# shenwei356/LexicMap

Measured on NVIDIA B200. Metric: aligned query bp/s, higher is better.
Workload: dtype int64

## Files before the change

lexicmap_b200/csrc/engine.cu:

```cuda
#include "image.cuh"
#include "../../include/lexicmap_gpu.h"
#include <cub/cub.cuh>
#include <cmath>
#include <cfloat>
#include <algorithm>
#include <numeric>
#include <chrono>
#include <mutex>
#include <atomic>
#include <thread>
#include <condition_variable>
#include <functional>
#include <exception>
#include <set>
#include <array>
#include <memory>
#include <sched.h>

#define FULLMASK 0xffffffffu
static std::atomic<unsigned long long> g_launches{0};
#undef KERNEL_CHECK
#define KERNEL_CHECK() do { g_launches++; CUDA_CHECK(cudaGetLastError()); } while (0)
#define CUB_CHECK() CUDA_CHECK(cudaGetLastError())
static inline int cdiv(i64 a, i64 b) { return (int)((a + b - 1) / b); }
// ... 838 lines not shown
    if (lane == 0) {
      R.wscore = s; i32 k = kend, off = tlen, sc = s; int mat = 0; i32 vv = off - k, h = off; u64* ops = (u64*)(slab + ((used + 1) & ~1ull)); u64 ops_room = (slab_words - ((used + 1) & ~1ull)) / 2; u32 nops = 0; bool ops_over = false;
      int cur = 0; u32 curn = 0; i32 p_alen = 0, p_gaps = 0, p_bs = 0; int prev = 0;
      auto flush = [&]() { if (want_ops && curn) { if (nops < ops_room) ops[nops++] = ((u64)cur << 32) | curn; else ops_over = true; } curn = 0; };
      auto put = [&](int op, i32 cntp, i32 vend, i32 hend) {
        if (cntp <= 0) return; if (op != cur) { flush(); cur = op; } curn += (u32)cntp;
        if (op == 'M') { if (R.has_m) { R.alen += p_alen; R.gaps += p_gaps; R.bscore += p_bs; } else { R.has_m = 1; R.qend = vend; R.tend = hend; } p_alen = p_gaps = p_bs = 0; R.alen += cntp; R.matches += cntp; R.bscore += 2 * cntp; R.qbegin = vend - cntp + 1; R.tbegin = hend - cntp + 1; }
        else if (op == 'X') { p_alen += cntp; p_bs -= 3 * cntp; } else { p_alen += cntp; p_gaps += cntp; p_bs -= 2 * cntp; if (prev != op) p_bs -= 5; }
        prev = op; };
      while (vv > 0 && h > 0 && sc > 0) {
        i32 s_mis = sc - X, s_open = sc - OE, s_ext = sc - E; i64 c_mis = INT64_MIN, c_io = INT64_MIN, c_ie = INT64_MIN, c_do = INT64_MIN, c_de = INT64_MIN;
        auto pig = [](i32 o, int type) -> i64 { return o <= WF_NULL ? INT64_MIN : (((i64)o << 4) | type); };
        if (mat == 0) { i32 o = (s_mis >= 0) ? getw(s_mis / STEP, 0, k) : WF_NULL; c_mis = pig(o <= WF_NULL ? WF_NULL : o + 1, 9); }
        if (mat == 0 || mat == 1) { i32 o = (s_open >= 0) ? getw(s_open / STEP, 0, k - 1) : WF_NULL; c_io = pig(o <= WF_NULL ? WF_NULL : o + 1, 1); o = (s_ext >= 0) ? getw(s_ext / STEP, 1, k - 1) : WF_NULL; c_ie = pig(o <= WF_NULL ? WF_NULL : o + 1, 2); }
        if (mat == 0 || mat == 2) { c_do = pig((s_open >= 0) ? getw(s_open / STEP, 0, k + 1) : WF_NULL, 5); c_de = pig((s_ext >= 0) ? getw(s_ext / STEP, 2, k + 1) : WF_NULL, 6); }
        i64 best = max(c_mis, max(max(c_io, c_ie), max(c_do, c_de))); if (best == INT64_MIN) { R.status = 2; break; }
        if (mat == 0) { i32 mo = (i32)(best >> 4); i32 nm = off - mo; put('M', nm, off - k, off); off = mo; vv = off - k; h = off; if (vv <= 0 || h <= 0) continue; }
        int type = (int)(best & 15);
        switch (type) { case 9: sc = s_mis; mat = 0; put('X', 1, off - k, off); off--; break;
          case 1: sc = s_open; mat = 0; put('I', 1, off - k, off); k--; off--; break; case 2: sc = s_ext; mat = 1; put('I', 1, off - k, off); k--; off--; break;
          case 5: sc = s_open; mat = 0; put('D', 1, off - k, off); k++; break; case 6: sc = s_ext; mat = 2; put('D', 1, off - k, off); k++; break; }
        vv = off - k; h = off;
      }
      if (R.status == 0) { if (sc == 0) put('M', off, off - k, off); else { if (vv > 0) put('D', vv, vv, h); if (h > 0) put('I', h, 0, h); } }
      flush();
      if (want_ops && R.status == 0) { if (ops_over) R.status = 1; else { u64 o = atomicAdd((unsigned long long*)ops_cursor, (unsigned long long)nops); if (o + nops <= ops_cap) { for (u32 i = 0; i < nops; i++) ops_pool[o + i] = ops[i]; R.ops_off = o; R.ops_n = nops; } else R.status = 3; } }
      outs[jb] = R;
    }
    __syncwarp();
  }
}

#define WF_WMAX 256
#define WF_PAD 8
#define WFS (WF_WMAX + 2 * WF_PAD)
#define WFK0 (WF_WMAX / 2 + WF_PAD)
#define WF_LMAX 2048
#define WF_OPSMAX 4096
#define WF_WARPS 8
#define WF_SEQW 144
#define X2_LV 2
#define OE2_LV 4
#define E2_LV 1
#define WF_SMEM_BYTES ((size_t)WF_WARPS * (WF_SEQW * 8 + 9 * WFS * 2 + WFS * 2))
struct WfaSeg { u64 qw, tw; };

__global__ void k_wfa_prep(const HspJob* __restrict__ jobs, const ExtOut* __restrict__ ext, u32 njobs, const u64* __restrict__ woff , const u8* __restrict__ qpacked, const u8* __restrict__ qamask, const u64* __restrict__ qboff,
                           const u8* __restrict__ g2bit, const u64* __restrict__ g_off, u64* __restrict__ words, u32* __restrict__ has_amb) {
  u32 jb = blockIdx.x; if (jb >= njobs) return; if (threadIdx.x == 0) has_amb[jb] = 0; __syncthreads(); HspJob J = jobs[jb]; ExtOut e = ext[jb]; const u8* q2 = qpacked + qboff[J.q]; const u8* qm = qamask + qboff[J.q]; const u8* g2 = g2bit + g_off[J.g];
  i32 plen = e.qe - e.qs, tlen = e.te - e.ts; u32 nq = (u32)((plen + 31) / 32 + 2), nt = (u32)((tlen + 31) / 32 + 2); u64* Q = words + woff[2 * jb]; u64* A = Q + nq; u64* T = words + woff[2 * jb + 1];
  for (u32 w = threadIdx.x; w < nq; w += blockDim.x) { u64 b = 0, a = 0; for (int j = 0; j < 32; j++) { i32 i = (i32)w * 32 + j; u64 c = 0, am = 0; if (i < plen) { i32 p = e.qs + i; c = get_base(q2, (u64)p); am = ((qm[p >> 3] >> (p & 7)) & 1) ? 3 : 0; } b = (b << 2) | c; a = (a << 2) | am; } Q[w] = b; A[w] = a; if (a) has_amb[jb] = 1; }
  for (u32 w = threadIdx.x; w < nt; w += blockDim.x) { u64 b = 0; for (int j = 0; j < 32; j++) { i32 i = (i32)w * 32 + j; u64 c = (i < tlen) ? win_base(g2, J.tBegin, J.tEnd, J.rc, e.ts + i) : 0; b = (b << 2) | c; } T[w] = b; }
}
__device__ __forceinline__ u64 fetch64(const u64* __restrict__ W, i32 pos) { u32 i = (u32)pos >> 5, sh = ((u32)pos & 31) * 2; u64 a = W[i]; if (sh == 0) return a; return (a << sh) | (W[i + 1] >> (64 - sh)); }

__global__ void __launch_bounds__(WF_WARPS * 32) k_wfa_fast(const ExtOut* __restrict__ ext, const u64* __restrict__ woff, const u64* __restrict__ words, const u32* __restrict__ has_amb, const u32* __restrict__ job_ids, u32 job0, u32 njobs, u32* __restrict__ next_job,
                                                          u16* __restrict__ slabs, WfaOut* __restrict__ outs, int adaptive, int lmax) {
  extern __shared__ __align__(16) u8 wf_smem[];
  const int X2 = 2, OE2 = 4, E2 = 1;
  int lane = threadIdx.x & 31, wib = threadIdx.x >> 5; u64* seqb = (u64*)wf_smem + (size_t)wib * WF_SEQW; u16 (*R)[WFS] = (u16 (*)[WFS])(wf_smem + (size_t)WF_WARPS * WF_SEQW * 8) + (size_t)wib * 9;
  u16* Dst = (u16*)(wf_smem + (size_t)WF_WARPS * WF_SEQW * 8 + (size_t)WF_WARPS * 9 * WFS * 2) + (size_t)wib * WFS;
  for (;;) {
    u32 jr = 0; if (lane == 0) jr = atomicAdd(next_job, 1u); jr = __shfl_sync(FULLMASK, jr, 0); if (jr >= njobs) return; const u32 jb = job_ids ? job_ids[job0 + jr] : job0 + jr; u16* slab = slabs + (u64)jr * lmax * 3 * WFS;
    ExtOut ex = ext[jb]; const i32 plen = ex.qe - ex.qs, tlen = ex.te - ex.ts, kend = tlen - plen; const u32 nqw = (u32)((plen + 31) / 32 + 2);
    const u64* Q = words + woff[2 * jb]; const u64* A = Q + nqw; const u64* T = words + woff[2 * jb + 1]; const bool amb = has_amb[jb] != 0;
    {
      const u32 ntw = (u32)((tlen + 31) / 32 + 2), nA = amb ? nqw : 0; __syncwarp();
      if (nqw + nA + ntw <= WF_SEQW) { u64* sq = seqb; for (u32 i = lane; i < nqw + nA; i += 32) sq[i] = Q[i]; for (u32 i = lane; i < ntw; i += 32) sq[nqw + nA + i] = T[i]; __syncwarp(); Q = sq; A = sq + nqw; T = sq + nqw + nA; } }
    WfaOut Rz; Rz.qbegin = Rz.qend = Rz.tbegin = Rz.tend = Rz.alen = Rz.matches = Rz.gaps = Rz.bscore = Rz.has_m = 0; Rz.wscore = 0; Rz.status = 0; Rz.ops_n = 0; Rz.ops_off = 0;
    if (plen >= 32000 || tlen >= 32000 || kend <= -(WF_WMAX / 2) + 2 || kend >= WF_WMAX / 2 - 2 || plen <= 0 || tlen <= 0) { if (lane == 0) { Rz.status = 1; outs[jb] = Rz; } __syncwarp(); continue; }
    auto extend = [&](i32 k, i32 h) { i32 v = h - k; for (;;) { i32 rem = min(plen - v, tlen - h); if (rem <= 0) break; u64 x = fetch64(Q, v) ^ fetch64(T, h); if (amb) x |= fetch64(A, v); i32 n = x ? (__clzll(x) >> 1) : 32; n = min(n, rem); v += n; h += n; if (n < 32) break; } return h; };
    i32 hlo[4], hhi[4]; u32 hnull[4]; for (int i = 0; i < 4; i++) { hlo[i] = 0; hhi[i] = -1; hnull[i] = 7; }
    for (int t = lane; t < 9 * WFS / 2; t += 32) ((u32*)&R[0][0])[t] = 0xFFFFFFFFu; __syncwarp();
    { i32 h0 = 0; if (lane == 0) h0 = extend(0, 0); h0 = __shfl_sync(FULLMASK, h0, 0);
      for (i32 k = -WF_PAD + lane; k <= WF_PAD; k += 32) { u16 mv = (k == 0) ? (u16)h0 : (u16)0xFFFF; R[0][k + WFK0] = mv; slab[k + WFK0] = mv; slab[WFS + k + WFK0] = 0xFFFF; slab[2 * WFS + k + WFK0] = 0xFFFF; R[5][k + WFK0] = 0xFFFF; R[7][k + WFK0] = 0xFFFF; }
      hlo[0] = 0; hhi[0] = 0; hnull[0] = 6; __syncwarp(); }
    i32 L = 0; bool done = (kend == 0 && R[0][WFK0] != 0xFFFF && (i32)R[0][WFK0] >= tlen), overflow = false;
    while (!done) {
      L++; if (L >= lmax) { overflow = true; break; }
      bool nx = (L - X2 < 0) || (hnull[X2 - 1] & 1), no = (L - OE2 < 0) || (hnull[OE2 - 1] & 1), ni = (hnull[E2 - 1] >> 1) & 1, nd = (hnull[E2 - 1] >> 2) & 1;
      i32 lo = INT32_MAX, hi = INT32_MIN; bool allnull = nx && no && ni && nd;
      if (!allnull) { if (!nx) { lo = min(lo, hlo[X2 - 1]); hi = max(hi, hhi[X2 - 1]); } if (!no) { lo = min(lo, hlo[OE2 - 1] - 1); hi = max(hi, hhi[OE2 - 1] + 1); } if (!ni || !nd) { lo = min(lo, hlo[E2 - 1] - 1); hi = max(hi, hhi[E2 - 1] + 1); } }
      i32 rlo = INT32_MAX, rhi = INT32_MIN; for (int i = 0; i < 4; i++) if (hnull[i] != 7) { rlo = min(rlo, hlo[i]); rhi = max(rhi, hhi[i]); }
      i32 wl = min(allnull ? INT32_MAX : lo, rlo), wh = max(allnull ? INT32_MIN : hi, rhi); if (wl > wh) { wl = 0; wh = 0; }
      if (wl <= -(WF_WMAX / 2) || wh >= WF_WMAX / 2) { overflow = true; break; }
      const u16* M2 = R[(L + 5 - X2) % 5]; const u16* M4 = R[(L + 5 - OE2) % 5]; const u16* I1 = R[5 + ((L + 1) & 1)]; const u16* D1 = R[7 + ((L + 1) & 1)];
      u16* Mo = R[L % 5]; u16* Io = R[5 + (L & 1)]; u16* Do = R[7 + (L & 1)]; u16* G = slab + (u64)L * 3 * WFS; bool anyM = false, anyI = false, anyD = false;
      u32 bitM = 0, bitI = 0, bitD = 0, itb = 1; i32 mind = INT32_MAX; const i32 k0 = wl - WF_PAD + lane;
      for (i32 k = k0; k <= wh + WF_PAD; k += 32, itb <<= 1) {
        u16 om = 0xFFFF, oi = 0xFFFF, od = 0xFFFF, dd = 0xFFFF; int x = k + WFK0;
        if (!allnull && k >= lo && k <= hi) {
          i32 ins = max((i32)(i16)M4[x - 1], (i32)(i16)I1[x - 1]); ins = (ins < 0) ? -1 : ins + 1;
          i32 del = max((i32)(i16)M4[x + 1], (i32)(i16)D1[x + 1]);
          i32 mis = (i32)(i16)M2[x]; mis = (mis < 0) ? -1 : mis + 1;
          const i32 hmax = min(tlen, plen + k);
          if (ins > hmax) ins = -1; if (del > hmax || del - k < 0) del = -1; if (mis > hmax) mis = -1;
          i32 mm = max(mis, max(ins, del)); if (mm >= 0) { mm = extend(k, mm); bitM |= itb; om = (u16)mm; i32 dv = max(plen - (mm - k), tlen - mm); dd = (u16)dv; mind = min(mind, dv); } if (ins >= 0) { bitI |= itb; oi = (u16)ins; } if (del >= 0) { bitD |= itb; od = (u16)del; }
        }
        Mo[x] = om; Io[x] = oi; Do[x] = od; Dst[x] = dd; G[x] = om; G[WFS + x] = oi; G[2 * WFS + x] = od;
      }
      anyM = __any_sync(FULLMASK, bitM != 0); anyI = __any_sync(FULLMASK, bitI != 0); anyD = __any_sync(FULLMASK, bitD != 0); __syncwarp();
      if (adaptive && !allnull && anyM && hi - lo + 1 >= 10) {
        for (int o = 16; o; o >>= 1) mind = min(mind, __shfl_xor_sync(FULLMASK, mind, o));
        const i32 thr = mind + 50; i32 top_limit = min(kend, hi); i32 nlo = lo; bool found = false;
        for (i32 b0 = lo; b0 < top_limit && !found; b0 += 32) { i32 k = b0 + lane; bool okk = (k < top_limit) && ((i32)Dst[k + WFK0] <= thr); u32 bal = __ballot_sync(FULLMASK, okk); if (bal) { nlo = b0 + __ffs(bal) - 1; found = true; } }
        if (!found && top_limit > lo) nlo = top_limit;
        i32 bottom_limit = max(kend, nlo); i32 nhi = hi; found = false;
        for (i32 b0 = hi; b0 > bottom_limit && !found; b0 -= 32) { i32 k = b0 - lane; bool okk = (k > bottom_limit) && ((i32)Dst[k + WFK0] <= thr); u32 bal = __ballot_sync(FULLMASK, okk); if (bal) { nhi = b0 - (__ffs(bal) - 1); found = true; } }
        if (!found && hi > bottom_limit) nhi = bottom_limit;
        if (nlo != lo || nhi != hi) { for (i32 k = lo + lane; k <= hi; k += 32) if (k < nlo || k > nhi) { int x = k + WFK0; Mo[x] = 0xFFFF; Io[x] = 0xFFFF; Do[x] = 0xFFFF; G[x] = 0xFFFF; G[WFS + x] = 0xFFFF; G[2 * WFS + x] = 0xFFFF; }
          i32 a0 = nlo - k0, a1 = nhi - k0; i32 itlo = a0 <= 0 ? 0 : (a0 + 31) >> 5, ithi = a1 < 0 ? -1 : (a1 >> 5); u32 keep = (ithi < itlo) ? 0u : ((ithi >= 31 ? 0xFFFFFFFFu : ((2u << ithi) - 1)) & ~((1u << itlo) - 1));
          anyM = __any_sync(FULLMASK, (bitM & keep) != 0); anyI = __any_sync(FULLMASK, (bitI & keep) != 0); anyD = __any_sync(FULLMASK, (bitD & keep) != 0); lo = nlo; hi = nhi; __syncwarp(); }
      }
      for (int i = 3; i > 0; i--) { hlo[i] = hlo[i - 1]; hhi[i] = hhi[i - 1]; hnull[i] = hnull[i - 1]; }
      hlo[0] = allnull ? 0 : lo; hhi[0] = allnull ? -1 : hi; hnull[0] = allnull ? 7u : ((anyM ? 0u : 1u) | (anyI ? 0u : 2u) | (anyD ? 0u : 4u));
      __syncwarp();
      if (!allnull && kend >= lo && kend <= hi) { u16 v = Mo[kend + WFK0]; done = (v != 0xFFFF && (i32)v >= tlen); }
    }
    if (lane == 0) { Rz.status = overflow ? 1 : 0; Rz.wscore = 2 * L; outs[jb] = Rz; }
    __syncwarp();
  }
}
__global__ void __launch_bounds__(128) k_wfa_bt(const ExtOut* __restrict__ ext, const u32* __restrict__ job_ids, u32 job0, u32 njobs, const u16* __restrict__ slabs, u64* __restrict__ ops_scratch, WfaOut* __restrict__ outs, u64* __restrict__ ops_pool, u64* __restrict__ ops_cursor, u64 ops_cap, int want_ops, int lmax) {
  const int X2 = 2, OE2 = 4, E2 = 1; u32 t = blockIdx.x * blockDim.x + threadIdx.x; if (t >= njobs) return; u32 jb = job_ids ? job_ids[job0 + t] : job0 + t; WfaOut Rr = outs[jb]; if (Rr.status != 0) return;
  ExtOut ex = ext[jb]; const i32 plen = ex.qe - ex.qs, tlen = ex.te - ex.ts, kend = tlen - plen; const u16* slab = slabs + (u64)t * lmax * 3 * WFS; u64* ops = ops_scratch + (u64)t * WF_OPSMAX;
  i32 L = Rr.wscore / 2; i32 k = kend, off = tlen, lv = L; int mat = 0; i32 vv = off - k, h = off; u32 nops = 0; bool ops_over = false; int cur = 0; u32 curn = 0; i32 p_alen = 0, p_gaps = 0, p_bs = 0; int prev = 0; (void)plen;
  auto flush = [&]() { if (want_ops && curn) { if (nops < WF_OPSMAX) ops[nops++] = ((u64)cur << 32) | curn; else ops_over = true; } curn = 0; };
  auto put = [&](int op, i32 cntp, i32 vend, i32 hend) { if (cntp <= 0) return; if (op != cur) { flush(); cur = op; } curn += (u32)cntp;
    if (op == 'M') { if (Rr.has_m) { Rr.alen += p_alen; Rr.gaps += p_gaps; Rr.bscore += p_bs; } else { Rr.has_m = 1; Rr.qend = vend; Rr.tend = hend; } p_alen = p_gaps = p_bs = 0; Rr.alen += cntp; Rr.matches += cntp; Rr.bscore += 2 * cntp; Rr.qbegin = vend - cntp + 1; Rr.tbegin = hend - cntp + 1; }
    else if (op == 'X') { p_alen += cntp; p_bs -= 3 * cntp; } else { p_alen += cntp; p_gaps += cntp; p_bs -= 2 * cntp; if (prev != op) p_bs -= 5; } prev = op; };
  auto ld = [&](i32 lvl, int comp, i32 kk) -> i32 { if (lvl < 0) return -1; u16 v = slab[(u64)lvl * 3 * WFS + comp * WFS + kk + WFK0]; return v == 0xFFFF ? -1 : (i32)v; };
  auto pig = [](i32 o, int type) -> i64 { return o < 0 ? INT64_MIN : (((i64)o << 4) | type); };
  while (vv > 0 && h > 0 && lv > 0) {
    i32 l_mis = lv - X2, l_open = lv - OE2, l_ext = lv - E2; i64 c_mis = INT64_MIN, c_io = INT64_MIN, c_ie = INT64_MIN, c_do = INT64_MIN, c_de = INT64_MIN;
    i32 v_mis = -1, v_io = -1, v_ie = -1, v_do = -1, v_de = -1;
    if (mat == 0) v_mis = ld(l_mis, 0, k); if (mat == 0 || mat == 1) { v_io = ld(l_open, 0, k - 1); v_ie = ld(l_ext, 1, k - 1); } if (mat == 0 || mat == 2) { v_do = ld(l_open, 0, k + 1); v_de = ld(l_ext, 2, k + 1); }
    if (mat == 0) c_mis = pig(v_mis < 0 ? -1 : v_mis + 1, 9); if (mat == 0 || mat == 1) { c_io = pig(v_io < 0 ? -1 : v_io + 1, 1); c_ie = pig(v_ie < 0 ? -1 : v_ie + 1, 2); } if (mat == 0 || mat == 2) { c_do = pig(v_do, 5); c_de = pig(v_de, 6); }
    i64 best = max(c_mis, max(max(c_io, c_ie), max(c_do, c_de))); if (best == INT64_MIN) { Rr.status = 2; break; }
    if (mat == 0) { i32 mo = (i32)(best >> 4); i32 nm = off - mo; put('M', nm, off - k, off); off = mo; vv = off - k; h = off; if (vv <= 0 || h <= 0) continue; }
    int type = (int)(best & 15);
    switch (type) { case 9: lv = l_mis; mat = 0; put('X', 1, off - k, off); off--; break;
      case 1: lv = l_open; mat = 0; put('I', 1, off - k, off); k--; off--; break; case 2: lv = l_ext; mat = 1; put('I', 1, off - k, off); k--; off--; break;
      case 5: lv = l_open; mat = 0; put('D', 1, off - k, off); k++; break; case 6: lv = l_ext; mat = 2; put('D', 1, off - k, off); k++; break; }
    vv = off - k; h = off;
  }
  if (Rr.status == 0) { if (lv == 0) put('M', off, off - k, off); else { if (vv > 0) put('D', vv, vv, h); if (h > 0) put('I', h, 0, h); } }
  flush();
  if (want_ops && Rr.status == 0) { if (ops_over) Rr.status = 1; else { u64 o = atomicAdd((unsigned long long*)ops_cursor, (unsigned long long)nops); if (o + nops <= ops_cap) { for (u32 i = 0; i < nops; i++) ops_pool[o + i] = ops[i]; Rr.ops_off = o; Rr.ops_n = nops; } else Rr.status = 3; } }
  outs[jb] = Rr;
}

#define WR_WARPS 8
#define WR_SEQW 144
#define WR_SMEM_BYTES ((size_t)WR_WARPS * WR_SEQW * 8)
#define WR_MAXLEN (1 << 20)
#define WR_NS 4
#define WR_W (32 * WR_NS)
struct WrCell { i32 om, oi, od, dv; u32 word; };
template <int NS>
__global__ void __launch_bounds__(WR_WARPS * 32) k_wfa_reg(const ExtOut* __restrict__ ext, const u64* __restrict__ woff, const u64* __restrict__ words, const u32* __restrict__ has_amb, const u32* __restrict__ job_ids, u32 job0, u32 njobs, u32* __restrict__ next_job,
                                                         u32* __restrict__ slabs, const u64* __restrict__ slab_off, WfaOut* __restrict__ outs, int adaptive) {
  extern __shared__ __align__(16) u8 wr_smem[];
  constexpr int W = 32 * NS;
  const int X2 = 2, OE2 = 4, E2 = 1; const int lane = threadIdx.x & 31, wib = threadIdx.x >> 5; u64* seqb = (u64*)wr_smem + (size_t)wib * WR_SEQW; const int lm1 = (lane + 31) & 31, lp1 = (lane + 1) & 31;
  for (;;) {
    u32 jr = 0; if (lane == 0) jr = atomicAdd(next_job, 1u); jr = __shfl_sync(FULLMASK, jr, 0); if (jr >= njobs) return; const u32 jb = job_ids ? job_ids[job0 + jr] : job0 + jr;
    u32* slab = slabs + slab_off[jr] * W; const i32 lmax = (i32)(slab_off[jr + 1] - slab_off[jr]);
    ExtOut ex = ext[jb]; const i32 plen = ex.qe - ex.qs, tlen = ex.te - ex.ts, kend = tlen - plen; const u32 nqw = (u32)((plen + 31) / 32 + 2);
    const u64* Q = words + woff[2 * jb]; const u64* A = Q + nqw; const u64* T = words + woff[2 * jb + 1]; const bool amb = has_amb[jb] != 0;
    { const u32 ntw = (u32)((tlen + 31) / 32 + 2), nA = amb ? nqw : 0; __syncwarp();
      if (nqw + nA + ntw <= WR_SEQW) { u64* sq = seqb; for (u32 i = lane; i < nqw + nA; i += 32) sq[i] = Q[i]; for (u32 i = lane; i < ntw; i += 32) sq[nqw + nA + i] = T[i]; __syncwarp(); Q = sq; A = sq + nqw; T = sq + nqw + nA; } }
    WfaOut Rz; Rz.qbegin = Rz.qend = Rz.tbegin = Rz.tend = Rz.alen = Rz.matches = Rz.gaps = Rz.bscore = Rz.has_m = 0; Rz.wscore = 0; Rz.status = 0; Rz.ops_n = 0; Rz.ops_off = 0;
    if (plen >= WR_MAXLEN || tlen >= WR_MAXLEN || plen <= 0 || tlen <= 0 || lmax < 2) { if (lane == 0) { Rz.status = 1; Rz.wscore = -3; outs[jb] = Rz; } __syncwarp(); continue; }
    auto extend = [&](i32 kk, i32 h) { i32 v = h - kk; for (;;) { i32 rem = min(plen - v, tlen - h); if (rem <= 0) break; u64 x = fetch64(Q, v) ^ fetch64(T, h); if (amb) x |= fetch64(A, v); i32 n = x ? (__clzll(x) >> 1) : 32; n = min(n, rem); v += n; h += n; if (n < 32) break; } return h; };
    auto cell = [&](i32 k, bool live, i32 c_m2, i32 m4l, i32 i1l, i32 m4r, i32 d1r) { WrCell c; c.om = -1; c.oi = -1; c.od = -1; c.dv = INT32_MAX; c.word = 0;
      if (live) { i32 ins = max(m4l, i1l); ins = (ins < 0) ? -1 : ins + 1; i32 del = max(m4r, d1r); i32 mis = (c_m2 < 0) ? -1 : c_m2 + 1;
        const i32 hmax = min(tlen, plen + k); if (ins > hmax) ins = -1; if (del > hmax || del - k < 0) del = -1; if (mis > hmax) mis = -1;
        i32 mm = max(mis, max(ins, del)); if (mm >= 0) { c.om = extend(k, mm); c.dv = max(plen - (c.om - k), tlen - c.om); } c.oi = ins; c.od = del;
        i32 best = -1; if (c_m2 >= 0) best = ((c_m2 + 1) << 4) | 9; if (m4l >= 0) best = max(best, ((m4l + 1) << 4) | 1); if (i1l >= 0) best = max(best, ((i1l + 1) << 4) | 2); if (m4r >= 0) best = max(best, (m4r << 4) | 5); if (d1r >= 0) best = max(best, (d1r << 4) | 6);
        if (best >= 0) c.word = (u32)(best >> 4) | ((u32)(best & 15) << 20);
        if (i1l >= 0 && i1l >= m4l) c.word |= 1u << 24; if (d1r >= 0 && d1r >= m4r) c.word |= 1u << 25; if (m4l < 0 && i1l < 0) c.word |= 1u << 26; if (m4r < 0 && d1r < 0) c.word |= 1u << 27; }
      return c; };
    i32 hlo[4], hhi[4]; u32 hnull[4]; for (int i = 0; i < 4; i++) { hlo[i] = 0; hhi[i] = -1; hnull[i] = 7; }
    i32 kb = -16;
    i32 m1[NS], m2[NS], m3[NS], m4[NS], i1[NS], d1[NS];
#pragma unroll
    for (int s_ = 0; s_ < NS; s_++) { m1[s_] = m2[s_] = m3[s_] = m4[s_] = i1[s_] = d1[s_] = -1; }
    if (kb + lane == 0) m1[0] = extend(0, 0); hlo[0] = 0; hhi[0] = 0; hnull[0] = 6; slab[lane] = lane == 0 ? (u32)kb : 0u;
    auto at = [&](const i32 (&v)[NS], i32 j) { i32 r = -1;
#pragma unroll
      for (int t = 0; t < NS; t++) { const i32 x = __shfl_sync(FULLMASK, v[t], j & 31); if ((j >> 5) == t) r = x; } return r; };
    i32 L = 0, why = 0; bool done = false, overflow = false; { const i32 v0 = at(m1, 0 - kb); done = (kend == 0 && v0 >= tlen); }
    while (!done) {
      L++; if (L >= lmax) { overflow = true; why = -1; break; }
      const bool nx = (L - X2 < 0) || (hnull[X2 - 1] & 1), no = (L - OE2 < 0) || (hnull[OE2 - 1] & 1), ni = (hnull[E2 - 1] >> 1) & 1, nd = (hnull[E2 - 1] >> 2) & 1;
      i32 lo = INT32_MAX, hi = INT32_MIN; const bool allnull = nx && no && ni && nd;
      if (!allnull) { if (!nx) { lo = min(lo, hlo[X2 - 1]); hi = max(hi, hhi[X2 - 1]); } if (!no) { lo = min(lo, hlo[OE2 - 1] - 1); hi = max(hi, hhi[OE2 - 1] + 1); } if (!ni || !nd) { lo = min(lo, hlo[E2 - 1] - 1); hi = max(hi, hhi[E2 - 1] + 1); } }
      i32 slo = allnull ? INT32_MAX : lo, shi = allnull ? INT32_MIN : hi; for (int i = 0; i < 4; i++) if (hnull[i] != 7) { slo = min(slo, hlo[i]); shi = max(shi, hhi[i]); }
      if (slo <= shi) { const i32 span = shi - slo + 1;
        if (slo < kb + 1 || shi > kb + W - 2 || (span <= 30 && shi > kb + 30)) { if (span > W - 2) { overflow = true; why = -2; break; }
          const i32 room = min(W - 2, ((span + 33) >> 5) * 32 - 2); const i32 nkb = slo - 1 - (room - span) / 2, dlt = nkb - kb;
          const int sl = (lane + (dlt & 31)) & 31, carry = (lane + (dlt & 31)) >> 5, q = dlt >> 5;
          auto shift = [&](i32 (&v)[NS]) { i32 x[NS];
#pragma unroll
            for (int t = 0; t < NS; t++) x[t] = __shfl_sync(FULLMASK, v[t], sl);
#pragma unroll
            for (int s_ = 0; s_ < NS; s_++) { const int src = s_ + q + carry; i32 r = -1;
#pragma unroll
              for (int t = 0; t < NS; t++) if (src == t) r = x[t]; v[s_] = r; } };
          shift(m1); shift(m2); shift(m3); shift(m4); shift(i1); shift(d1); kb = nkb; } }
      const int sa = (slo <= shi) ? max(0, (slo - kb) >> 5) : 0, sb = (slo <= shi) ? min(NS - 1, (shi - kb) >> 5) : -1;
      WrCell c[NS];
#pragma unroll
      for (int s_ = 0; s_ < NS; s_++) { c[s_].om = c[s_].oi = c[s_].od = -1; c[s_].dv = INT32_MAX; c[s_].word = 0; }
      if (!allnull) {
        i32 r4[NS], ri[NS], t4[NS], td[NS];
#pragma unroll
        for (int t = 0; t < NS; t++) { r4[t] = ri[t] = t4[t] = td[t] = -1; if (t >= sa && t <= sb) { r4[t] = __shfl_sync(FULLMASK, m4[t], lm1); ri[t] = __shfl_sync(FULLMASK, i1[t], lm1); t4[t] = __shfl_sync(FULLMASK, m4[t], lp1); td[t] = __shfl_sync(FULLMASK, d1[t], lp1); } }
#pragma unroll
        for (int s_ = 0; s_ < NS; s_++) if (s_ >= sa && s_ <= sb && lo <= kb + 32 * s_ + 31 && hi >= kb + 32 * s_) { const i32 k = kb + 32 * s_ + lane;
            const i32 l4 = lane ? r4[s_] : (s_ ? r4[s_ - 1] : -1), li = lane ? ri[s_] : (s_ ? ri[s_ - 1] : -1), g4 = lane < 31 ? t4[s_] : (s_ < NS - 1 ? t4[s_ + 1] : -1), gd = lane < 31 ? td[s_] : (s_ < NS - 1 ? td[s_ + 1] : -1);
            c[s_] = cell(k, k >= lo && k <= hi, m2[s_], l4, li, g4, gd); } }
      bool hm = false, hi_ = false, hd = false;
#pragma unroll
      for (int s_ = 0; s_ < NS; s_++) { hm |= c[s_].om >= 0; hi_ |= c[s_].oi >= 0; hd |= c[s_].od >= 0; }
      bool anyM = __any_sync(FULLMASK, hm), anyI = __any_sync(FULLMASK, hi_), anyD = __any_sync(FULLMASK, hd);
      if (adaptive && !allnull && anyM && hi - lo + 1 >= 10) {
        i32 mind = INT32_MAX;
#pragma unroll
        for (int s_ = 0; s_ < NS; s_++) mind = min(mind, c[s_].dv);
        for (int o = 16; o; o >>= 1) mind = min(mind, __shfl_xor_sync(FULLMASK, mind, o)); const i32 thr = mind + 50;
        const i32 top_limit = min(kend, hi); i32 nlo = lo; bool found = false;
#pragma unroll
        for (int s_ = 0; s_ < NS; s_++) if (s_ >= sa && s_ <= sb) { const i32 k = kb + 32 * s_ + lane; const u32 bal = __ballot_sync(FULLMASK, c[s_].om >= 0 && c[s_].dv <= thr && k >= lo && k < top_limit); if (bal && !found) { nlo = kb + 32 * s_ + __ffs(bal) - 1; found = true; } }
        if (!found && top_limit > lo) nlo = top_limit;
        const i32 bottom_limit = max(kend, nlo); i32 nhi = hi; found = false;
#pragma unroll
        for (int s_ = NS - 1; s_ >= 0; s_--) if (s_ >= sa && s_ <= sb) { const i32 k = kb + 32 * s_ + lane; const u32 bal = __ballot_sync(FULLMASK, c[s_].om >= 0 && c[s_].dv <= thr && k <= hi && k > bottom_limit); if (bal && !found) { nhi = kb + 32 * s_ + 31 - __clz(bal); found = true; } }
        if (!found && hi > bottom_limit) nhi = bottom_limit;
        if (nlo != lo || nhi != hi) { hm = hi_ = hd = false;
#pragma unroll
          for (int s_ = 0; s_ < NS; s_++) { const i32 k = kb + 32 * s_ + lane; if (k < nlo || k > nhi) { c[s_].om = -1; c[s_].oi = -1; c[s_].od = -1; } hm |= c[s_].om >= 0; hi_ |= c[s_].oi >= 0; hd |= c[s_].od >= 0; }
          anyM = __any_sync(FULLMASK, hm); anyI = __any_sync(FULLMASK, hi_); anyD = __any_sync(FULLMASK, hd); lo = nlo; hi = nhi; }
      }
      { u32* row = slab + (u64)L * W;
#pragma unroll
        for (int s_ = 0; s_ < NS; s_++) if (s_ == 0 || (s_ >= sa && s_ <= sb)) row[32 * s_ + lane] = (s_ == 0 && lane == 0) ? (u32)kb : c[s_].word; }
#pragma unroll
      for (int s_ = 0; s_ < NS; s_++) { m4[s_] = m3[s_]; m3[s_] = m2[s_]; m2[s_] = m1[s_]; m1[s_] = c[s_].om; i1[s_] = c[s_].oi; d1[s_] = c[s_].od; }
      for (int i = 3; i > 0; i--) { hlo[i] = hlo[i - 1]; hhi[i] = hhi[i - 1]; hnull[i] = hnull[i - 1]; }
      hlo[0] = allnull ? 0 : lo; hhi[0] = allnull ? -1 : hi; hnull[0] = allnull ? 7u : ((anyM ? 0u : 1u) | (anyI ? 0u : 2u) | (anyD ? 0u : 4u));
      if (!allnull && kend >= lo && kend <= hi) { const i32 v = at(m1, kend - kb); done = (v >= tlen); }
    }
    if (lane == 0) { Rz.status = overflow ? 1 : 0; Rz.wscore = overflow ? why : 2 * L; outs[jb] = Rz; }
    __syncwarp();
  }
}
__global__ void __launch_bounds__(128) k_wfa_bt2(const ExtOut* __restrict__ ext, const u32* __restrict__ job_ids, u32 job0, u32 njobs, const u32* __restrict__ slabs, const u64* __restrict__ slab_off, u64* __restrict__ ops_scratch, const u64* __restrict__ ops_off, WfaOut* __restrict__ outs, u64* __restrict__ ops_pool, u64* __restrict__ ops_cursor, u64 ops_cap, int want_ops, int W) {
  u32 t = blockIdx.x * blockDim.x + threadIdx.x; if (t >= njobs) return; u32 jb = job_ids ? job_ids[job0 + t] : job0 + t; WfaOut Rr = outs[jb]; if (Rr.status != 0) return;
  ExtOut ex = ext[jb]; const i32 plen = ex.qe - ex.qs, tlen = ex.te - ex.ts, kend = tlen - plen; const u32* slab = slabs + slab_off[t] * W; u64* ops = ops_scratch + (want_ops ? ops_off[t] : 0); const u32 ops_max = want_ops ? (u32)(ops_off[t + 1] - ops_off[t]) : 0;
  i32 k = kend, off = tlen, lv = Rr.wscore / 2; int mat = 0; i32 vv = off - k, h = off; u32 nops = 0; bool ops_over = false; int cur = 0; u32 curn = 0; i32 p_alen = 0, p_gaps = 0, p_bs = 0; int prev = 0;
  auto flush = [&]() { if (want_ops && curn) { if (nops < ops_max) ops[nops++] = ((u64)cur << 32) | curn; else ops_over = true; } curn = 0; };
  auto put = [&](int op, i32 cntp, i32 vend, i32 hend) { if (cntp <= 0) return; if (op != cur) { flush(); cur = op; } curn += (u32)cntp;
    if (op == 'M') { if (Rr.has_m) { Rr.alen += p_alen; Rr.gaps += p_gaps; Rr.bscore += p_bs; } else { Rr.has_m = 1; Rr.qend = vend; Rr.tend = hend; } p_alen = p_gaps = p_bs = 0; Rr.alen += cntp; Rr.matches += cntp; Rr.bscore += 2 * cntp; Rr.qbegin = vend - cntp + 1; Rr.tbegin = hend - cntp + 1; }
    else if (op == 'X') { p_alen += cntp; p_bs -= 3 * cntp; } else { p_alen += cntp; p_gaps += cntp; p_bs -= 2 * cntp; if (prev != op) p_bs -= 5; } prev = op; };
  while (vv > 0 && h > 0 && lv > 0) {
    const u32* row = slab + (u64)lv * W; const i32 kb = (i32)row[0]; const u32 li = (u32)(k - kb); if (li - 1u > (u32)(W - 3)) { Rr.status = 2; break; } const u32 cell = row[li]; int type;
    if (mat == 0) { type = (int)((cell >> 20) & 15); if (type == 0) { Rr.status = 2; break; } const i32 mo = (i32)(cell & 0xFFFFF); put('M', off - mo, off - k, off); off = mo; vv = off - k; h = off; if (vv <= 0 || h <= 0) continue; }
    else if (mat == 1) { if ((cell >> 26) & 1) { Rr.status = 2; break; } type = ((cell >> 24) & 1) ? 2 : 1; }
    else { if ((cell >> 27) & 1) { Rr.status = 2; break; } type = ((cell >> 25) & 1) ? 6 : 5; }
    switch (type) { case 9: lv -= X2_LV; mat = 0; put('X', 1, off - k, off); off--; break;
      case 1: lv -= OE2_LV; mat = 0; put('I', 1, off - k, off); k--; off--; break; case 2: lv -= E2_LV; mat = 1; put('I', 1, off - k, off); k--; off--; break;
      case 5: lv -= OE2_LV; mat = 0; put('D', 1, off - k, off); k++; break; case 6: lv -= E2_LV; mat = 2; put('D', 1, off - k, off); k++; break; default: Rr.status = 2; break; }
    if (Rr.status) break; vv = off - k; h = off;
  }
  if (Rr.status == 0) { if (lv == 0) put('M', off, off - k, off); else { if (vv > 0) put('D', vv, vv, h); if (h > 0) put('I', h, 0, h); } }
  flush();
  if (want_ops && Rr.status == 0) { if (ops_over) Rr.status = 1; else { u64 o = atomicAdd((unsigned long long*)ops_cursor, (unsigned long long)nops); if (o + nops <= ops_cap) { for (u32 i = 0; i < nops; i++) ops_pool[o + i] = ops[i]; Rr.ops_off = o; Rr.ops_n = nops; } else Rr.status = 3; } }
  (void)plen; outs[jb] = Rr;
}

static void wfa_raise_smem_limit() { static std::mutex mu; static std::set<int> done; int dev = 0; CUDA_CHECK(cudaGetDevice(&dev)); std::lock_guard<std::mutex> lk(mu); if (done.count(dev)) return;
  CUDA_CHECK(cudaFuncSetAttribute(k_wfa_fast, cudaFuncAttributeMaxDynamicSharedMemorySize, (int)WF_SMEM_BYTES)); done.insert(dev); }
static void wfa_run_all(cudaStream_t st, int sm_count, DBuf<HspJob>& d_jobs, DBuf<ExtOut>& d_ext, const std::vector<ExtOut>& hext, u32 nj, const u8* qpacked, const u8* qamask, const u64* qboff, const u8* g2bit, const u64* g_off,
                        int want_ops, int adaptive, std::vector<WfaOut>& hw, std::vector<u64>& hops, u64* counters, double* ms, size_t total_mem, int active_lanes = 1) {
    wfa_raise_smem_limit();
    DBuf<WfaOut> d_out(nj, st); std::vector<u32> ids; hw.resize(nj);
    u64 ops_cap = 0; if (want_ops) { for (u32 j = 0; j < nj; j++) ops_cap += (u64)(hext[j].qe - hext[j].qs) + (hext[j].te - hext[j].ts) + 4; } DBuf<u64> ops_pool(ops_cap + 2, st); DBuf<u64> ops_cur(1, st); ops_cur.zero();
    DBuf<u64> woff, words; DBuf<u32> hasamb;
    { std::vector<u64> hwoff(2 * (u64)nj + 1, 0); for (u32 j = 0; j < nj; j++) { u64 nqw = (u64)((hext[j].qe - hext[j].qs + 31) / 32 + 2), ntw = (u64)((hext[j].te - hext[j].ts + 31) / 32 + 2); hwoff[2 * j + 1] = hwoff[2 * j] + 2 * nqw; hwoff[2 * j + 2] = hwoff[2 * j + 1] + ntw; }
      woff.alloc(hwoff.size(), st); woff.from_host(hwoff.data(), hwoff.size()); words.alloc(hwoff.back() + 4, st); hasamb.alloc(nj + 1, st);
      if (g_lap) (*g_lap)("wfa host prep"); { KTimer kt(st, &ms[10]); k_wfa_prep<<<nj, 64, 0, st>>>(d_jobs.p, d_ext.p, nj, woff.p, qpacked, qamask, qboff, g2bit, g_off, words.p, hasamb.p); KERNEL_CHECK(); }
      i32 maxlen = 1; for (u32 j = 0; j < nj; j++) maxlen = std::max(maxlen, std::max(hext[j].qe - hext[j].qs, hext[j].te - hext[j].ts));
      const int lmax = (int)std::min<i64>(WF_LMAX * 2, std::max<i64>(256, ((i64)(0.8 * maxlen) + 63) / 64 * 64));
      const size_t tb_ = total_mem; const u64 budgetF = std::min<u64>((u64)(tb_ * 0.25), 36ull << 30) / (u64)std::max(1, active_lanes);
      if (g_lap) (*g_lap)("wfa prep kernel");
      std::vector<u32> rest;
      static const bool use_reg = getenv("LMG_NO_WFA_REG") == nullptr;
      if (use_reg) {
        auto lv_cap = [&](u32 j) { const i64 len = std::max(hext[j].qe - hext[j].qs, hext[j].te - hext[j].ts); return (u64)std::max<i64>(256, ((i64)(0.8 * (double)len) + 63) / 64 * 64); };
        auto op_cap = [&](u32 j) { const i64 len = std::max(hext[j].qe - hext[j].qs, hext[j].te - hext[j].ts); return want_ops ? (u64)std::max<i64>(1024, len + 64) : 0ull; };
        std::vector<u32> skipped; u32 round_max = 0; std::vector<i32> len(nj); for (u32 j = 0; j < nj; j++) len[j] = std::max(hext[j].qe - hext[j].qs, hext[j].te - hext[j].ts);
        auto run_reg = [&](const std::vector<u32>& ord, int NS, std::vector<u32>& skip) { const u32 cnt = (u32)ord.size(); const u64 W = 32ull * (u64)NS; std::vector<u64> hso, hoo; DBuf<u32> d_order(cnt, st); d_order.from_host(ord.data(), cnt);
          KTimer kt(st, &ms[11]);
          for (u32 j0 = 0; j0 < cnt;) { hso.assign(1, 0); hoo.assign(1, 0); u64 bytes = 0; u32 n = 0;
// ... 410 lines not shown
```

Measured before the change: 116.5 million.

## Add single-segment fast path and 32-bit staged extend to register WFA kernel

The register-resident WFA kernel gains a fast path for when the active diagonal band fits in the first 32-lane segment. That path computes a single cell per lane and skips the multi-segment shuffles and loops. Status flags (M/I/D presence and done) are folded into one warp OR-reduction, replacing three __any_sync calls and a shuffle-based lookup. Staged sequences are word-swapped so the extend step can use 32-bit funnel-shift fetches from shared memory, and fetch64 becomes branchless. Launch bounds add a minimum-blocks hint, which may force register spills in the NS=4 instantiation.

```diff
diff --git a/lexicmap_b200/csrc/engine.cu b/lexicmap_b200/csrc/engine.cu
--- a/lexicmap_b200/csrc/engine.cu
+++ b/lexicmap_b200/csrc/engine.cu
@@ -914,7 +914,7 @@
   for (u32 w = threadIdx.x; w < nq; w += blockDim.x) { u64 b = 0, a = 0; for (int j = 0; j < 32; j++) { i32 i = (i32)w * 32 + j; u64 c = 0, am = 0; if (i < plen) { i32 p = e.qs + i; c = get_base(q2, (u64)p); am = ((qm[p >> 3] >> (p & 7)) & 1) ? 3 : 0; } b = (b << 2) | c; a = (a << 2) | am; } Q[w] = b; A[w] = a; if (a) has_amb[jb] = 1; }
   for (u32 w = threadIdx.x; w < nt; w += blockDim.x) { u64 b = 0; for (int j = 0; j < 32; j++) { i32 i = (i32)w * 32 + j; u64 c = (i < tlen) ? win_base(g2, J.tBegin, J.tEnd, J.rc, e.ts + i) : 0; b = (b << 2) | c; } T[w] = b; }
 }
-__device__ __forceinline__ u64 fetch64(const u64* __restrict__ W, i32 pos) { u32 i = (u32)pos >> 5, sh = ((u32)pos & 31) * 2; u64 a = W[i]; if (sh == 0) return a; return (a << sh) | (W[i + 1] >> (64 - sh)); }
+__device__ __forceinline__ u64 fetch64(const u64* __restrict__ W, i32 pos) { u32 i = (u32)pos >> 5, sh = ((u32)pos & 31) * 2; u64 a = W[i], b = W[i + 1]; return (a << sh) | ((b >> 1) >> (63 - sh)); }
 
 __global__ void __launch_bounds__(WF_WARPS * 32) k_wfa_fast(const ExtOut* __restrict__ ext, const u64* __restrict__ woff, const u64* __restrict__ words, const u32* __restrict__ has_amb, const u32* __restrict__ job_ids, u32 job0, u32 njobs, u32* __restrict__ next_job,
                                                           u16* __restrict__ slabs, WfaOut* __restrict__ outs, int adaptive, int lmax) {
@@ -1019,8 +1019,19 @@
 #define WR_NS 4
 #define WR_W (32 * WR_NS)
 struct WrCell { i32 om, oi, od, dv; u32 word; };
+__device__ __forceinline__ u32 fetchw(const u32* __restrict__ S, i32 pos) { const u32 j = (u32)pos >> 4; return __funnelshift_l(S[j + 1], S[j], ((u32)pos & 15) * 2); }
+__device__ __forceinline__ u64 fetchw(const u64* __restrict__ W, i32 pos) { return fetch64(W, pos); }
+template <typename Wd>
+__device__ __forceinline__ i32 wr_extend(const Wd* __restrict__ Q, const Wd* __restrict__ A, const Wd* __restrict__ T, bool amb, i32 plen, i32 tlen, i32 kk, i32 h) {
+  constexpr i32 B = 4 * sizeof(Wd);
+  i32 v = h - kk; for (;;) { i32 rem = min(plen - v, tlen - h); if (rem <= 0) break; Wd x = fetchw(Q, v) ^ fetchw(T, h); if (amb) x |= fetchw(A, v); i32 n = (B == 32 ? __clzll((u64)x) : __clz((u32)x)) >> 1; n = min(n, rem); v += n; h += n; if (n < B) break; }
+  return h; }
+#define WR_FM 1u
+#define WR_FI 2u
+#define WR_FD 4u
+#define WR_FDONE 8u
 template <int NS>
-__global__ void __launch_bounds__(WR_WARPS * 32) k_wfa_reg(const ExtOut* __restrict__ ext, const u64* __restrict__ woff, const u64* __restrict__ words, const u32* __restrict__ has_amb, const u32* __restrict__ job_ids, u32 job0, u32 njobs, u32* __restrict__ next_job,
+__global__ void __launch_bounds__(WR_WARPS * 32, NS == 4 ? 4 : 2) k_wfa_reg(const ExtOut* __restrict__ ext, const u64* __restrict__ woff, const u64* __restrict__ words, const u32* __restrict__ has_amb, const u32* __restrict__ job_ids, u32 job0, u32 njobs, u32* __restrict__ next_job,
                                                          u32* __restrict__ slabs, const u64* __restrict__ slab_off, WfaOut* __restrict__ outs, int adaptive) {
   extern __shared__ __align__(16) u8 wr_smem[];
   constexpr int W = 32 * NS;
@@ -1030,11 +1041,14 @@
     u32* slab = slabs + slab_off[jr] * W; const i32 lmax = (i32)(slab_off[jr + 1] - slab_off[jr]);
     ExtOut ex = ext[jb]; const i32 plen = ex.qe - ex.qs, tlen = ex.te - ex.ts, kend = tlen - plen; const u32 nqw = (u32)((plen + 31) / 32 + 2);
     const u64* Q = words + woff[2 * jb]; const u64* A = Q + nqw; const u64* T = words + woff[2 * jb + 1]; const bool amb = has_amb[jb] != 0;
-    { const u32 ntw = (u32)((tlen + 31) / 32 + 2), nA = amb ? nqw : 0; __syncwarp();
-      if (nqw + nA + ntw <= WR_SEQW) { u64* sq = seqb; for (u32 i = lane; i < nqw + nA; i += 32) sq[i] = Q[i]; for (u32 i = lane; i < ntw; i += 32) sq[nqw + nA + i] = T[i]; __syncwarp(); Q = sq; A = sq + nqw; T = sq + nqw + nA; } }
+    const u32 ntw = (u32)((tlen + 31) / 32 + 2), nA = amb ? nqw : 0; const bool staged = nqw + nA + ntw <= WR_SEQW;
+    __syncwarp();
+    if (staged) { auto sw = [](u64 w) { return (w << 32) | (w >> 32); };
+      for (u32 i = lane; i < nqw + nA; i += 32) seqb[i] = sw(Q[i]); for (u32 i = lane; i < ntw; i += 32) seqb[nqw + nA + i] = sw(T[i]); __syncwarp(); }
     WfaOut Rz; Rz.qbegin = Rz.qend = Rz.tbegin = Rz.tend = Rz.alen = Rz.matches = Rz.gaps = Rz.bscore = Rz.has_m = 0; Rz.wscore = 0; Rz.status = 0; Rz.ops_n = 0; Rz.ops_off = 0;
     if (plen >= WR_MAXLEN || tlen >= WR_MAXLEN || plen <= 0 || tlen <= 0 || lmax < 2) { if (lane == 0) { Rz.status = 1; Rz.wscore = -3; outs[jb] = Rz; } __syncwarp(); continue; }
-    auto extend = [&](i32 kk, i32 h) { i32 v = h - kk; for (;;) { i32 rem = min(plen - v, tlen - h); if (rem <= 0) break; u64 x = fetch64(Q, v) ^ fetch64(T, h); if (amb) x |= fetch64(A, v); i32 n = x ? (__clzll(x) >> 1) : 32; n = min(n, rem); v += n; h += n; if (n < 32) break; } return h; };
+    const u32* sq = (const u32*)seqb;
+    auto extend = [&](i32 kk, i32 h) { return staged ? wr_extend(sq, sq + 2 * nqw, sq + 2 * (nqw + nA), amb, plen, tlen, kk, h) : wr_extend(Q, A, T, amb, plen, tlen, kk, h); };
     auto cell = [&](i32 k, bool live, i32 c_m2, i32 m4l, i32 i1l, i32 m4r, i32 d1r) { WrCell c; c.om = -1; c.oi = -1; c.od = -1; c.dv = INT32_MAX; c.word = 0;
       if (live) { i32 ins = max(m4l, i1l); ins = (ins < 0) ? -1 : ins + 1; i32 del = max(m4r, d1r); i32 mis = (c_m2 < 0) ? -1 : c_m2 + 1;
         const i32 hmax = min(tlen, plen + k); if (ins > hmax) ins = -1; if (del > hmax || del - k < 0) del = -1; if (mis > hmax) mis = -1;
@@ -1043,24 +1057,40 @@
         if (best >= 0) c.word = (u32)(best >> 4) | ((u32)(best & 15) << 20);
         if (i1l >= 0 && i1l >= m4l) c.word |= 1u << 24; if (d1r >= 0 && d1r >= m4r) c.word |= 1u << 25; if (m4l < 0 && i1l < 0) c.word |= 1u << 26; if (m4r < 0 && d1r < 0) c.word |= 1u << 27; }
       return c; };
+    auto flags = [&](const WrCell& c, i32 k) { return (c.om >= 0 ? WR_FM : 0u) | (c.oi >= 0 ? WR_FI : 0u) | (c.od >= 0 ? WR_FD : 0u) | (k == kend && c.om >= tlen ? WR_FDONE : 0u); };
     i32 hlo[4], hhi[4]; u32 hnull[4]; for (int i = 0; i < 4; i++) { hlo[i] = 0; hhi[i] = -1; hnull[i] = 7; }
     i32 kb = -16;
     i32 m1[NS], m2[NS], m3[NS], m4[NS], i1[NS], d1[NS];
 #pragma unroll
     for (int s_ = 0; s_ < NS; s_++) { m1[s_] = m2[s_] = m3[s_] = m4[s_] = i1[s_] = d1[s_] = -1; }
     if (kb + lane == 0) m1[0] = extend(0, 0); hlo[0] = 0; hhi[0] = 0; hnull[0] = 6; slab[lane] = lane == 0 ? (u32)kb : 0u;
-    auto at = [&](const i32 (&v)[NS], i32 j) { i32 r = -1;
-#pragma unroll
-      for (int t = 0; t < NS; t++) { const i32 x = __shfl_sync(FULLMASK, v[t], j & 31); if ((j >> 5) == t) r = x; } return r; };
-    i32 L = 0, why = 0; bool done = false, overflow = false; { const i32 v0 = at(m1, 0 - kb); done = (kend == 0 && v0 >= tlen); }
+    i32 L = 0, why = 0; bool done = __any_sync(FULLMASK, kb + lane == kend && m1[0] >= tlen), overflow = false;
     while (!done) {
       L++; if (L >= lmax) { overflow = true; why = -1; break; }
       const bool nx = (L - X2 < 0) || (hnull[X2 - 1] & 1), no = (L - OE2 < 0) || (hnull[OE2 - 1] & 1), ni = (hnull[E2 - 1] >> 1) & 1, nd = (hnull[E2 - 1] >> 2) & 1;
       i32 lo = INT32_MAX, hi = INT32_MIN; const bool allnull = nx && no && ni && nd;
       if (!allnull) { if (!nx) { lo = min(lo, hlo[X2 - 1]); hi = max(hi, hhi[X2 - 1]); } if (!no) { lo = min(lo, hlo[OE2 - 1] - 1); hi = max(hi, hhi[OE2 - 1] + 1); } if (!ni || !nd) { lo = min(lo, hlo[E2 - 1] - 1); hi = max(hi, hhi[E2 - 1] + 1); } }
       i32 slo = allnull ? INT32_MAX : lo, shi = allnull ? INT32_MIN : hi; for (int i = 0; i < 4; i++) if (hnull[i] != 7) { slo = min(slo, hlo[i]); shi = max(shi, hhi[i]); }
-      if (slo <= shi) { const i32 span = shi - slo + 1;
-        if (slo < kb + 1 || shi > kb + W - 2 || (span <= 30 && shi > kb + 30)) { if (span > W - 2) { overflow = true; why = -2; break; }
+      u32 fl;
+      u32* row = slab + (u64)L * W;
+      const bool moved = slo <= shi && (slo < kb + 1 || shi > kb + W - 2 || (shi - slo + 1 <= 30 && shi > kb + 30));
+      if (!moved && (slo > shi || shi < kb + 32)) {
+        const i32 k = kb + lane;
+        const i32 l4 = __shfl_sync(FULLMASK, m4[0], lm1), li = __shfl_sync(FULLMASK, i1[0], lm1), g4 = __shfl_sync(FULLMASK, m4[0], lp1), gd = __shfl_sync(FULLMASK, d1[0], lp1);
+        WrCell c = cell(k, k >= lo && k <= hi, m2[0], lane ? l4 : -1, lane ? li : -1, lane < 31 ? g4 : -1, lane < 31 ? gd : -1);
+        fl = __reduce_or_sync(FULLMASK, flags(c, k));
+        if (adaptive && !allnull && (fl & WR_FM) && hi - lo + 1 >= 10) {
+          const i32 thr = __reduce_min_sync(FULLMASK, c.dv) + 50; const bool ok = c.om >= 0 && c.dv <= thr;
+          const i32 top_limit = min(kend, hi); i32 nlo = lo;
+          u32 bal = __ballot_sync(FULLMASK, ok && k >= lo && k < top_limit); if (bal) nlo = kb + __ffs(bal) - 1; else if (top_limit > lo) nlo = top_limit;
+          const i32 bottom_limit = max(kend, nlo); i32 nhi = hi;
+          bal = __ballot_sync(FULLMASK, ok && k <= hi && k > bottom_limit); if (bal) nhi = kb + 31 - __clz(bal); else if (hi > bottom_limit) nhi = bottom_limit;
+          if (nlo != lo || nhi != hi) { if (k < nlo || k > nhi) { c.om = -1; c.oi = -1; c.od = -1; } fl = __reduce_or_sync(FULLMASK, flags(c, k)); lo = nlo; hi = nhi; }
+        }
+        row[lane] = lane == 0 ? (u32)kb : c.word;
+        m4[0] = m3[0]; m3[0] = m2[0]; m2[0] = m1[0]; m1[0] = c.om; i1[0] = c.oi; d1[0] = c.od;
+      } else {
+        if (moved) { const i32 span = shi - slo + 1; if (span > W - 2) { overflow = true; why = -2; break; }
           const i32 room = min(W - 2, ((span + 33) >> 5) * 32 - 2); const i32 nkb = slo - 1 - (room - span) / 2, dlt = nkb - kb;
           const int sl = (lane + (dlt & 31)) & 31, carry = (lane + (dlt & 31)) >> 5, q = dlt >> 5;
           auto shift = [&](i32 (&v)[NS]) { i32 x[NS];
@@ -1070,49 +1100,49 @@
             for (int s_ = 0; s_ < NS; s_++) { const int src = s_ + q + carry; i32 r = -1;
 #pragma unroll
               for (int t = 0; t < NS; t++) if (src == t) r = x[t]; v[s_] = r; } };
-          shift(m1); shift(m2); shift(m3); shift(m4); shift(i1); shift(d1); kb = nkb; } }
-      const int sa = (slo <= shi) ? max(0, (slo - kb) >> 5) : 0, sb = (slo <= shi) ? min(NS - 1, (shi - kb) >> 5) : -1;
-      WrCell c[NS];
+          shift(m1); shift(m2); shift(m3); shift(m4); shift(i1); shift(d1); kb = nkb; }
+        const int sa = (slo <= shi) ? max(0, (slo - kb) >> 5) : 0, sb = (slo <= shi) ? min(NS - 1, (shi - kb) >> 5) : -1;
+        WrCell c[NS];
 #pragma unroll
-      for (int s_ = 0; s_ < NS; s_++) { c[s_].om = c[s_].oi = c[s_].od = -1; c[s_].dv = INT32_MAX; c[s_].word = 0; }
-      if (!allnull) {
-        i32 r4[NS], ri[NS], t4[NS], td[NS];
+        for (int s_ = 0; s_ < NS; s_++) { c[s_].om = c[s_].oi = c[s_].od = -1; c[s_].dv = INT32_MAX; c[s_].word = 0; }
+        if (!allnull) {
+          i32 r4[NS], ri[NS], t4[NS], td[NS];
 #pragma unroll
-        for (int t = 0; t < NS; t++) { r4[t] = ri[t] = t4[t] = td[t] = -1; if (t >= sa && t <= sb) { r4[t] = __shfl_sync(FULLMASK, m4[t], lm1); ri[t] = __shfl_sync(FULLMASK, i1[t], lm1); t4[t] = __shfl_sync(FULLMASK, m4[t], lp1); td[t] = __shfl_sync(FULLMASK, d1[t], lp1); } }
+          for (int t = 0; t < NS; t++) { r4[t] = ri[t] = t4[t] = td[t] = -1; if (t >= sa && t <= sb) { r4[t] = __shfl_sync(FULLMASK, m4[t], lm1); ri[t] = __shfl_sync(FULLMASK, i1[t], lm1); t4[t] = __shfl_sync(FULLMASK, m4[t], lp1); td[t] = __shfl_sync(FULLMASK, d1[t], lp1); } }
 #pragma unroll
-        for (int s_ = 0; s_ < NS; s_++) if (s_ >= sa && s_ <= sb && lo <= kb + 32 * s_ + 31 && hi >= kb + 32 * s_) { const i32 k = kb + 32 * s_ + lane;
-            const i32 l4 = lane ? r4[s_] : (s_ ? r4[s_ - 1] : -1), li = lane ? ri[s_] : (s_ ? ri[s_ - 1] : -1), g4 = lane < 31 ? t4[s_] : (s_ < NS - 1 ? t4[s_ + 1] : -1), gd = lane < 31 ? td[s_] : (s_ < NS - 1 ? td[s_ + 1] : -1);
-            c[s_] = cell(k, k >= lo && k <= hi, m2[s_], l4, li, g4, gd); } }
-      bool hm = false, hi_ = false, hd = false;
+          for (int s_ = 0; s_ < NS; s_++) if (s_ >= sa && s_ <= sb && lo <= kb + 32 * s_ + 31 && hi >= kb + 32 * s_) { const i32 k = kb + 32 * s_ + lane;
+              const i32 l4 = lane ? r4[s_] : (s_ ? r4[s_ - 1] : -1), li = lane ? ri[s_] : (s_ ? ri[s_ - 1] : -1), g4 = lane < 31 ? t4[s_] : (s_ < NS - 1 ? t4[s_ + 1] : -1), gd = lane < 31 ? td[s_] : (s_ < NS - 1 ? td[s_ + 1] : -1);
+              c[s_] = cell(k, k >= lo && k <= hi, m2[s_], l4, li, g4, gd); } }
+        u32 f = 0;
 #pragma unroll
-      for (int s_ = 0; s_ < NS; s_++) { hm |= c[s_].om >= 0; hi_ |= c[s_].oi >= 0; hd |= c[s_].od >= 0; }
-      bool anyM = __any_sync(FULLMASK, hm), anyI = __any_sync(FULLMASK, hi_), anyD = __any_sync(FULLMASK, hd);
-      if (adaptive && !allnull && anyM && hi - lo + 1 >= 10) {
-        i32 mind = INT32_MAX;
+        for (int s_ = 0; s_ < NS; s_++) f |= flags(c[s_], kb + 32 * s_ + lane);
+        fl = __reduce_or_sync(FULLMASK, f);
+        if (adaptive && !allnull && (fl & WR_FM) && hi - lo + 1 >= 10) {
+          i32 mind = INT32_MAX;
 #pragma unroll
-        for (int s_ = 0; s_ < NS; s_++) mind = min(mind, c[s_].dv);
-        for (int o = 16; o; o >>= 1) mind = min(mind, __shfl_xor_sync(FULLMASK, mind, o)); const i32 thr = mind + 50;
-        const i32 top_limit = min(kend, hi); i32 nlo = lo; bool found = false;
+          for (int s_ = 0; s_ < NS; s_++) mind = min(mind, c[s_].dv);
+          const i32 thr = __reduce_min_sync(FULLMASK, mind) + 50;
+          const i32 top_limit = min(kend, hi); i32 nlo = lo; bool found = false;
 #pragma unroll
-        for (int s_ = 0; s_ < NS; s_++) if (s_ >= sa && s_ <= sb) { const i32 k = kb + 32 * s_ + lane; const u32 bal = __ballot_sync(FULLMASK, c[s_].om >= 0 && c[s_].dv <= thr && k >= lo && k < top_limit); if (bal && !found) { nlo = kb + 32 * s_ + __ffs(bal) - 1; found = true; } }
-        if (!found && top_limit > lo) nlo = top_limit;
-        const i32 bottom_limit = max(kend, nlo); i32 nhi = hi; found = false;
+          for (int s_ = 0; s_ < NS; s_++) if (s_ >= sa && s_ <= sb) { const i32 k = kb + 32 * s_ + lane; const u32 bal = __ballot_sync(FULLMASK, c[s_].om >= 0 && c[s_].dv <= thr && k >= lo && k < top_limit); if (bal && !found) { nlo = kb + 32 * s_ + __ffs(bal) - 1; found = true; } }
+          if (!found && top_limit > lo) nlo = top_limit;
+          const i32 bottom_limit = max(kend, nlo); i32 nhi = hi; found = false;
 #pragma unroll
-        for (int s_ = NS - 1; s_ >= 0; s_--) if (s_ >= sa && s_ <= sb) { const i32 k = kb + 32 * s_ + lane; const u32 bal = __ballot_sync(FULLMASK, c[s_].om >= 0 && c[s_].dv <= thr && k <= hi && k > bottom_limit); if (bal && !found) { nhi = kb + 32 * s_ + 31 - __clz(bal); found = true; } }
-        if (!found && hi > bottom_limit) nhi = bottom_limit;
-        if (nlo != lo || nhi != hi) { hm = hi_ = hd = false;
+          for (int s_ = NS - 1; s_ >= 0; s_--) if (s_ >= sa && s_ <= sb) { const i32 k = kb + 32 * s_ + lane; const u32 bal = __ballot_sync(FULLMASK, c[s_].om >= 0 && c[s_].dv <= thr && k <= hi && k > bottom_limit); if (bal && !found) { nhi = kb + 32 * s_ + 31 - __clz(bal); found = true; } }
+          if (!found && hi > bottom_limit) nhi = bottom_limit;
+          if (nlo != lo || nhi != hi) { f = 0;
 #pragma unroll
-          for (int s_ = 0; s_ < NS; s_++) { const i32 k = kb + 32 * s_ + lane; if (k < nlo || k > nhi) { c[s_].om = -1; c[s_].oi = -1; c[s_].od = -1; } hm |= c[s_].om >= 0; hi_ |= c[s_].oi >= 0; hd |= c[s_].od >= 0; }
-          anyM = __any_sync(FULLMASK, hm); anyI = __any_sync(FULLMASK, hi_); anyD = __any_sync(FULLMASK, hd); lo = nlo; hi = nhi; }
+            for (int s_ = 0; s_ < NS; s_++) { const i32 k = kb + 32 * s_ + lane; if (k < nlo || k > nhi) { c[s_].om = -1; c[s_].oi = -1; c[s_].od = -1; } f |= flags(c[s_], k); }
+            fl = __reduce_or_sync(FULLMASK, f); lo = nlo; hi = nhi; }
+        }
+#pragma unroll
+        for (int s_ = 0; s_ < NS; s_++) if (s_ == 0 || (s_ >= sa && s_ <= sb)) row[32 * s_ + lane] = (s_ == 0 && lane == 0) ? (u32)kb : c[s_].word;
+#pragma unroll
+        for (int s_ = 0; s_ < NS; s_++) { m4[s_] = m3[s_]; m3[s_] = m2[s_]; m2[s_] = m1[s_]; m1[s_] = c[s_].om; i1[s_] = c[s_].oi; d1[s_] = c[s_].od; }
       }
-      { u32* row = slab + (u64)L * W;
-#pragma unroll
-        for (int s_ = 0; s_ < NS; s_++) if (s_ == 0 || (s_ >= sa && s_ <= sb)) row[32 * s_ + lane] = (s_ == 0 && lane == 0) ? (u32)kb : c[s_].word; }
-#pragma unroll
-      for (int s_ = 0; s_ < NS; s_++) { m4[s_] = m3[s_]; m3[s_] = m2[s_]; m2[s_] = m1[s_]; m1[s_] = c[s_].om; i1[s_] = c[s_].oi; d1[s_] = c[s_].od; }
       for (int i = 3; i > 0; i--) { hlo[i] = hlo[i - 1]; hhi[i] = hhi[i - 1]; hnull[i] = hnull[i - 1]; }
-      hlo[0] = allnull ? 0 : lo; hhi[0] = allnull ? -1 : hi; hnull[0] = allnull ? 7u : ((anyM ? 0u : 1u) | (anyI ? 0u : 2u) | (anyD ? 0u : 4u));
-      if (!allnull && kend >= lo && kend <= hi) { const i32 v = at(m1, kend - kb); done = (v >= tlen); }
+      hlo[0] = allnull ? 0 : lo; hhi[0] = allnull ? -1 : hi; hnull[0] = allnull ? 7u : (((fl & WR_FM) ? 0u : 1u) | ((fl & WR_FI) ? 0u : 2u) | ((fl & WR_FD) ? 0u : 4u));
+      done = (fl & WR_FDONE) != 0;
     }
     if (lane == 0) { Rz.status = overflow ? 1 : 0; Rz.wscore = overflow ? why : 2 * L; outs[jb] = Rz; }
     __syncwarp();
```

After: 119.2 million, median of 6. +2.3%, better.
